# tyiannak/pyAudioAnalysis

Measured on AMD Instinct MI355X. Metric: short-term frames/sec (34-feat, 16 kHz, 50 ms/25 ms) + HBM GB/s vs peak, higher is better.
Workload: dtype f64

## Files before the change

include/paa_hip.h:

```cpp
#ifndef PAA_HIP_H
#define PAA_HIP_H

#include <stddef.h>
#include <stdint.h>

#ifdef __cplusplus
extern "C" {
#endif

#define PAA_OK                 0
#define PAA_ERR_ARG          (-1)
#define PAA_ERR_UNSUPPORTED  (-2)
#define PAA_ERR_HIP          (-3)
#define PAA_ERR_OOM          (-4)
#define PAA_ERR_TOO_SHORT    (-5)
#define PAA_ERR_CHROMA_VALUE (-6)
#define PAA_ERR_CHROMA_INDEX (-7)
#define PAA_ERR_MEL_INDEX    (-8)
#define PAA_ERR_COMM         (-9)

#define PAA_N_BASE_FEATURES 34

const char *paa_version(void);
const char *paa_last_error(void);
// ... 193 lines not shown
int paa_lda_dev_project_f64(const double *d_x, int n_dims, int64_t ld, int64_t n_vec, const double *xbar, const double *scalings,
                            int n_out, double *d_y, int64_t ld_y);

#define PAA_COMM_ID_BYTES 128
int paa_comm_unique_id(void *id_out );
int paa_comm_init(int world_size, int rank, const void *id);
int paa_comm_destroy(void);
int paa_comm_gather_f64(const double *d_send, const int64_t *counts, int root, double *d_recv);
int paa_comm_gatherv_f64(const double *d_send, const int64_t *counts, const int64_t *displs, int root, double *d_recv);
int paa_comm_barrier(void);

int paa_debug_mel_bank(double fs, int num_fft, double *out_dense);
int paa_debug_dct(double *out_13x40);
int paa_debug_chroma(double fs, int num_fft, int capacity, int32_t *src, double *weight, int32_t *slot);
int paa_debug_plan_clip_norms(paa_plan_t *plan, const void *d_packed, double *out, int64_t capacity);
int paa_debug_wave_trace(uint64_t *out, int max_waves);
int paa_debug_lane_peak(void);
int paa_debug_phase_cycles(uint64_t *out16);
int paa_debug_fft_plan(int window, int32_t *radices, int32_t *fft_len);
int paa_debug_comm_marker_name(const void *unique_id, int rank, char *out, int capacity);
int paa_debug_tri_plan(int window, double fs, int32_t *shape8, int32_t *offsets6, unsigned char *blob, int capacity);
int paa_debug_wg_plan(int window, int32_t *info32, uint16_t *perm, int perm_capacity);
int paa_debug_wgs_plan(int window, int32_t *info16, int32_t *bin_of, int capacity);
int paa_debug_wgr_tables(double fs, int window, int32_t *mel_job, int32_t *mel_fil, int32_t *ch_n, int32_t *ch_src, double *ch_w);
int paa_debug_wgr_runs(const int64_t *frames, int64_t n_clips, int num_cu, int32_t *runs3, int64_t capacity, int64_t *n_runs);
int paa_debug_blu_plan(int window, double fs, int32_t *info8, int32_t *offsets3, unsigned char *blob, int capacity);
int paa_debug_lane_jobs(const int32_t *first, const int32_t *wfirst, const int32_t *cnt, int n_owners, int32_t *jobs256);
int paa_debug_mix_plan(int window, int32_t *radices, int32_t *fft_len, uint16_t *perm, int perm_capacity,
                       int32_t *waves, int32_t *tw_global);
int paa_debug_run_plan(const int64_t *frames, int64_t n_clips, int quantum, int min_run, int max_run, int halo, int wg_runs,
// ... 11 lines not shown
```

pyaudioanalysis_amd/_ffi.py:

```python
import ctypes as C
import os
import threading

import numpy as np

from . import _build

PAA_OK = 0
ERR_ARG, ERR_UNSUPPORTED, ERR_HIP, ERR_OOM = -1, -2, -3, -4
ERR_TOO_SHORT, ERR_CHROMA_VALUE, ERR_CHROMA_INDEX, ERR_MEL_INDEX, ERR_COMM = -5, -6, -7, -8, -9
COMM_ID_BYTES = 128

_lock = threading.Lock()
_lib = None

c_i16p = C.POINTER(C.c_int16)
c_f64p = C.POINTER(C.c_double)
c_i64p = C.POINTER(C.c_int64)
c_i32p = C.POINTER(C.c_int32)


class HipLibraryError(RuntimeError):
    """libpaa_hip.so is missing / unbuildable, or the HIP runtime reported an error."""

# ... 133 lines not shown
    "paa_lda_dev_project_f64": (C.c_int, [C.c_void_p, C.c_int, C.c_int64, C.c_int64, c_f64p, c_f64p, C.c_int, C.c_void_p,
                                          C.c_int64]),
    "paa_comm_unique_id": (C.c_int, [C.c_void_p]),
    "paa_comm_init": (C.c_int, [C.c_int, C.c_int, C.c_void_p]),
    "paa_comm_destroy": (C.c_int, []),
    "paa_comm_gather_f64": (C.c_int, [C.c_void_p, c_i64p, C.c_int, C.c_void_p]),
    "paa_comm_gatherv_f64": (C.c_int, [C.c_void_p, c_i64p, c_i64p, C.c_int, C.c_void_p]),
    "paa_comm_barrier": (C.c_int, []),
    "paa_debug_mel_bank": (C.c_int, [C.c_double, C.c_int, c_f64p]),
    "paa_debug_dct": (C.c_int, [c_f64p]),
    "paa_debug_chroma": (C.c_int, [C.c_double, C.c_int, C.c_int, c_i32p, c_f64p, c_i32p]),
    "paa_debug_plan_clip_norms": (C.c_int, [C.c_void_p, C.c_void_p, c_f64p, C.c_int64]),
    "paa_debug_phase_cycles": (C.c_int, [C.POINTER(C.c_uint64)]),
    "paa_debug_wave_trace": (C.c_int, [C.POINTER(C.c_uint64), C.c_int]),
    "paa_debug_lane_peak": (C.c_int, []),
    "paa_debug_fft_plan": (C.c_int, [C.c_int, c_i32p, c_i32p]),
    "paa_debug_comm_marker_name": (C.c_int, [C.c_void_p, C.c_int, C.c_char_p, C.c_int]),
    "paa_debug_tri_plan": (C.c_int, [C.c_int, C.c_double, c_i32p, c_i32p, C.c_void_p, C.c_int]),
    "paa_debug_wg_plan": (C.c_int, [C.c_int, c_i32p, C.POINTER(C.c_uint16), C.c_int]),
    "paa_debug_wgs_plan": (C.c_int, [C.c_int, c_i32p, c_i32p, C.c_int]),
    "paa_debug_wgr_tables": (C.c_int, [C.c_double, C.c_int, c_i32p, c_i32p, c_i32p, c_i32p, c_f64p]),
    "paa_debug_wgr_runs": (C.c_int, [c_i64p, C.c_int64, C.c_int, c_i32p, C.c_int64, c_i64p]),
    "paa_debug_blu_plan": (C.c_int, [C.c_int, C.c_double, c_i32p, c_i32p, C.c_void_p, C.c_int]),
    "paa_debug_lane_jobs": (C.c_int, [c_i32p, c_i32p, c_i32p, C.c_int, c_i32p]),
    "paa_debug_mix_plan": (C.c_int, [C.c_int, c_i32p, c_i32p, C.POINTER(C.c_uint16), C.c_int, c_i32p, c_i32p]),
    "paa_debug_run_plan": (C.c_int, [c_i64p, C.c_int64, C.c_int, C.c_int, C.c_int, C.c_int, C.c_int, C.c_int, c_i32p,
                                     c_i64p, c_i32p]),
    "paa_debug_run_plan_shrink": (C.c_int, [c_i64p, C.c_int64, C.c_int, C.c_int, C.c_int, C.c_int, C.c_int, C.c_int, c_i32p,
                                     c_i64p, c_i32p]),
    "paa_debug_balanced_runs": (C.c_int64, [c_i64p, C.c_int64, C.c_int, C.c_int, C.c_int, C.c_int, C.c_int, C.c_int, c_i32p,
# ... 230 lines not shown
```

pyaudioanalysis_amd/csrc/comm_rccl.hpp:

```cpp
#pragma once
#include <dirent.h>
#include <fcntl.h>
#include <signal.h>
#include <sys/stat.h>
#include <unistd.h>

#include <rccl/rccl.h>

namespace {
struct RcclApi {
    void *h = nullptr;
    ncclResult_t (*GetUniqueId)(ncclUniqueId *) = nullptr;
    ncclResult_t (*CommInitRank)(ncclComm_t *, int, ncclUniqueId, int) = nullptr;
    ncclResult_t (*CommDestroy)(ncclComm_t) = nullptr;
    ncclResult_t (*Send)(const void *, size_t, ncclDataType_t, int, ncclComm_t, hipStream_t) = nullptr;
    ncclResult_t (*Recv)(void *, size_t, ncclDataType_t, int, ncclComm_t, hipStream_t) = nullptr;
    ncclResult_t (*GroupStart)() = nullptr;
    ncclResult_t (*GroupEnd)() = nullptr;
    ncclResult_t (*AllReduce)(const void *, void *, size_t, ncclDataType_t, ncclRedOp_t, ncclComm_t, hipStream_t) = nullptr;
    const char *(*GetErrorString)(ncclResult_t) = nullptr;
};
RcclApi g_rccl;
ncclComm_t g_comm = nullptr;
int g_world = 1, g_rank = 0;
// ... 179 lines not shown
    if (g_comm_stream) { (void)hipStreamDestroy(g_comm_stream); g_comm_stream = nullptr; }
    if (g_bar) { (void)hipFree(g_bar); g_bar = nullptr; }
    comm_release_device();
    g_world = 1;
    g_rank = 0;
    return PAA_OK;
}

extern "C" int paa_comm_gatherv_f64(const double *d_send, const int64_t *counts, const int64_t *displs, int root,
                                    double *d_recv) {
    if (!counts || !displs) return fail(PAA_ERR_ARG, "null counts / displs");
    std::lock_guard<std::mutex> lk(g_mu);
    if (!g_comm) {
        if (g_world != 1) return fail(PAA_ERR_COMM, "communicator not initialised");
        if (d_recv && d_send && d_recv + displs[0] != d_send && counts[0] > 0)
            HIP_TRY(hipMemcpyAsync(d_recv + displs[0], d_send, (size_t)counts[0] * 8, hipMemcpyDeviceToDevice, g_main_stream));
        return PAA_OK;
    }
    if (root < 0 || root >= g_world) return fail(PAA_ERR_ARG, "bad root");
    if (g_rank == root && !d_recv) return fail(PAA_ERR_ARG, "root needs a receive buffer");
    HIP_TRY(hipEventRecord(g_ev_ready, g_main_stream));
    HIP_TRY(hipStreamWaitEvent(g_comm_stream, g_ev_ready, 0));
    NCCL_TRY(g_rccl.GroupStart());
    ncclResult_t in_group = ncclSuccess;
    if (g_rank == root) {
        for (int r = 0; r < g_world && in_group == ncclSuccess; ++r)
            if (r != root && counts[r] > 0)
                in_group = g_rccl.Recv(d_recv + displs[r], (size_t)counts[r], ncclDouble, r, g_comm, g_comm_stream);
    } else if (counts[g_rank] > 0) {
        if (!d_send) in_group = ncclInvalidArgument;
        else in_group = g_rccl.Send(d_send, (size_t)counts[g_rank], ncclDouble, root, g_comm, g_comm_stream);
    }
    const ncclResult_t at_end = g_rccl.GroupEnd();
    if (in_group != ncclSuccess) return fail(PAA_ERR_COMM, "ncclSend / ncclRecv of the gather: %s", g_rccl.GetErrorString(in_group));
    if (at_end != ncclSuccess) return fail(PAA_ERR_COMM, "ncclGroupEnd of the gather: %s", g_rccl.GetErrorString(at_end));
    if (g_rank == root && d_send && counts[root] > 0 && d_recv + displs[root] != d_send)
// ... 26 lines not shown
        else (void)hipGetLastError();
        for (auto it = g_gather_done.begin(); it != g_gather_done.end();) {
            const char *k = static_cast<const char *>(it->first);
            if (k >= lo && k < hi) {
                if (it->second) gone.push_back(it->second);
                it = g_gather_done.erase(it);
            } else {
                ++it;
            }
        }
    }
    for (hipEvent_t ev : gone) { (void)hipEventSynchronize(ev); (void)hipEventDestroy(ev); }
}
static hipStream_t comm_stream_or_null() { return g_comm ? g_comm_stream : nullptr; }
static int comm_order_after_compute(hipStream_t s) {
    HIP_TRY(hipEventRecord(g_ev_ready, g_main_stream));
    HIP_TRY(hipStreamWaitEvent(s, g_ev_ready, 0));
    return PAA_OK;
}
static int comm_wait_buffer_free(const void *d_out) {
    auto it = g_gather_done.find(d_out);
    if (it != g_gather_done.end() && it->second) HIP_TRY(hipStreamWaitEvent(g_main_stream, it->second, 0));
    return PAA_OK;
}
static int comm_sync() {
    if (g_comm_stream) HIP_TRY(hipStreamSynchronize(g_comm_stream));
    return PAA_OK;
}

extern "C" int paa_comm_barrier(void) {
    if (!g_comm) return PAA_OK;
    HIP_TRY(hipStreamSynchronize(g_main_stream));
    NCCL_TRY(g_rccl.AllReduce(g_bar, g_bar, 1, ncclInt, ncclSum, g_comm, g_comm_stream));
    HIP_TRY(hipStreamSynchronize(g_comm_stream));
    return PAA_OK;
}
```

pyaudioanalysis_amd/csrc/lib_debug.hpp:

```cpp
#pragma once
extern "C" int paa_debug_phase_cycles(uint64_t *out16) {
    if (!out16) return fail(PAA_ERR_ARG, "null");
    for (int i = 0; i < 16; ++i) out16[i] = 0;
#if defined(PAA_F800_TIMING) || defined(PAA_F800_TRACE)
    int rc = ensure_init();
    if (rc) return rc;
    HIP_TRY(hipStreamSynchronize(cs()));
    unsigned long long acc[16] = {0};
    if (launch::phase_fast(acc, nullptr, 0) < 0 || launch::phase_ct(acc, nullptr, 0) < 0 || launch::phase_tri_a(acc, nullptr, 0) < 0 ||
        launch::phase_tri_b(acc, nullptr, 0) < 0 || launch::phase_tri_c(acc, nullptr, 0) < 0 || launch::phase_rmg(acc, nullptr, 0) < 0 || launch::phase_blu(acc, nullptr, 0) < 0 ||
        launch::phase_wgr(acc, nullptr, 0) < 0)
        return fail(PAA_ERR_HIP, "reading the phase counters failed");
    for (int i = 0; i < 16; ++i) out16[i] = acc[i];
#endif
    return PAA_OK;
}

extern "C" int paa_debug_lane_peak(void) {
    std::lock_guard<std::mutex> lk(g_lane_mu);
    const int p = g_lanes_peak;
    g_lanes_peak = g_lanes_active;
    return p;
}

// ... 10 lines not shown
#else
    return 0;
#endif
}

extern "C" int paa_debug_plan_clip_norms(paa_plan_t *plan, const void *d_packed, double *out, int64_t capacity) {
    if (!plan || !d_packed || !out) return fail(PAA_ERR_ARG, "null plan / buffer");
    if (capacity < 10 * (plan->n_clips + 1))
        return fail(PAA_ERR_ARG, "capacity %lld < %lld doubles", (long long)capacity, 10LL * (plan->n_clips + 1));
    { const int rc_init = ensure_init(); if (rc_init) return rc_init; }
    std::lock_guard<std::mutex> lk(g_mu);
    const int rc = launch_stats(plan, d_packed, true);
    if (rc) return rc;
    HIP_TRY(hipStreamSynchronize(cs()));
    std::vector<ClipNorm> nm((size_t)plan->n_clips);
    HIP_TRY(hipMemcpy(nm.data(), plan->d_norms, nm.size() * sizeof(ClipNorm), hipMemcpyDeviceToHost));
    const double head[10] = {(double)plan->stat_chunk, (double)g_num_cu, (double)plan->n_clips, (double)plan->n_chunks,
                             (double)plan->P.norms_inline, (double)plan->sample_kind, 0.0, 0.0, 0.0, 0.0};
    std::copy(head, head + 10, out);
    for (long long c = 0; c < plan->n_clips; ++c) {
        const ClipNorm &n = nm[(size_t)c];
        const double row[10] = {n.mean, n.inv, n.mu, n.delta_mu, (double)n.m_int, (double)n.zb, (double)n.mu_whole, n.dc_shift,
                                (double)plan->clips[c].stat_first, (double)plan->clips[c].stat_count};
        std::copy(row, row + 10, out + 10 * (c + 1));
    }
    return PAA_OK;
}

extern "C" int paa_debug_mel_bank(double fs, int num_fft, double *out_dense) {
    if (!out_dense || num_fft < 1) return fail(PAA_ERR_ARG, "bad argument");
    MelTable t;
    int rc = build_mel(fs, num_fft, t);
    if (rc) return fail(rc, "mel filter bank indexes bin >= num_fft");
    std::fill(out_dense, out_dense + (size_t)kNumMel * num_fft, 0.0);
    for (int m = 0; m < kNumMel; ++m)
        for (int i = 0; i < t.cnt[m]; ++i) out_dense[(size_t)m * num_fft + t.lo[m] + i] = t.w[t.off[m] + i];
    return PAA_OK;
}
extern "C" int paa_debug_dct(double *out_13x40) {
    if (!out_13x40) return fail(PAA_ERR_ARG, "null");
    build_dct(out_13x40);
// ... 219 lines not shown
```

pyaudioanalysis_amd/csrc/lib_dispatch.hpp:

```cpp
#pragma once

struct FamilyCtx {
    paa_plan *p;
    TableSet *tab;
    double fs;
    int window, step, deltas, mode, sample_kind, F;
    long long total_frames;
    int ranges;
    int num_cu() const { return g_num_cu * (ranges > 1 ? ranges : 1); }
    const MelTable *mel() const { return mode == 0 ? &tab->mel : nullptr; }
    const ChromaTable *chroma() const { return mode != 1 ? &tab->chroma : nullptr; }
};
struct RunRule {
    int run = 64, quantum = 4, halo_inside = 0;
    int fill_wg_runs = 0;
    int fill_min_run = 16;
};
struct Family {
    const char *id;
    int (*select)(const FamilyCtx &c, FamilyChoice &f, std::vector<unsigned char> &blob);
    int (*work)(FamilyCtx &c, std::vector<Tile> &tiles);
    int (*execute)(paa_plan *p, const void *d_packed, double *d_out, const Tile *tiles, long long n_tiles);
    bool ranged;
    bool norms_inline;
// ... 40 lines not shown
    }
}
template <void (*Rule)(FamilyCtx &, RunRule &)>
static int tile_work(FamilyCtx &c, std::vector<Tile> &tiles) {
    RunRule rr;
    Rule(c, rr);
    build_tiles(c, rr, tiles);
    return PAA_OK;
}
typedef int (*TileLaunch)(const paa_plan *p, const TileArgs &a);
template <TileLaunch Launch>
static int tile_execute(paa_plan *p, const void *d_packed, double *d_out, const Tile *tiles, long long n_tiles) {
    if (n_tiles == 0) return PAA_OK;
    ProfScope prof_scope;
    { const int rc_p = prof_scope.begin(); if (rc_p) return rc_p; }
    const TileArgs a{p->P, p->fam.d_blob, d_packed, p->sample_kind, p->d_clips, p->d_norms, tiles, n_tiles, d_out, cs()};
    return Launch(p, a) ? launch_failed(p) : PAA_OK;
}

static int fam_fast_select(const FamilyCtx &c, FamilyChoice &f, std::vector<unsigned char> &) {
    if (c.mode != 0 || g_force_generic) return 0;
    const int rc = fast_select(c.window, c.step, c.sample_kind, c.fs, c.tab->fast, c.tab->fft, c.tab->mel, c.tab->chroma, f.fl,
                               g_f800_waves);
    if (rc < 0) return fail(rc, "building the tables of the specialised kernel failed");
    if (rc) { f.lds = f.fl.lds; f.kernel_name = f.fl.name; }
    return rc;
}
static void fam_fast_rule(FamilyCtx &c, RunRule &r) {
    const FastLaunch &fl = c.p->fam.fl;
    r.quantum = 4;
    r.halo_inside = c.deltas ? 2 : 1;
// ... 158 lines not shown
                        wg::FrameRef f = p->wg_frames[(size_t)i];
                        f.halo |= q << 8;
                        p->wg_tasks.push_back(f);
                    }
            p->wg_task_chunks.emplace_back(t0, (long long)p->wg_tasks.size());
        }
    } else {
        return PAA_OK;
    }
    if (p->wg_tasks.size() > 0x7fffffffULL) return fail(PAA_ERR_UNSUPPORTED, "too many frames for the split transform");
    return upload_pooled(&p->d_wg_tasks, p->wg_tasks.data(), std::max<size_t>(p->wg_tasks.size(), 1));
}
static int fam_wgs_work(FamilyCtx &c, std::vector<Tile> &) { return wg_build_work(c.p, wgs::wgs_select(c.window).r0); }
static int fam_wg_work(FamilyCtx &c, std::vector<Tile> &) { return wg_build_work(c.p, 0); }
static WgArgs wg_args(const paa_plan *p, const void *d_packed, double *d_out) {
    return WgArgs{p->P, d_packed, p->sample_kind, p->d_clips, p->d_norms, d_out, g_num_cu, cs()};
}
static int fam_wgr_execute(paa_plan *p, const void *d_packed, double *d_out, const Tile *runs, long long n_runs) {
    return run_wgr(p, wg_args(p, d_packed, d_out), runs, n_runs);
}
static int fam_wgs_execute(paa_plan *p, const void *d_packed, double *d_out, const Tile *, long long) {
    return run_wgs(p, wg_args(p, d_packed, d_out), wgs::wgs_select(p->P.W));
}
static int fam_wg_execute(paa_plan *p, const void *d_packed, double *d_out, const Tile *, long long) {
    const WgArgs a = wg_args(p, d_packed, d_out);
    return with_sample_type(p->sample_kind, [&](auto tag) {
        typedef PAA_SAMPLE_T(tag) T;
        wg_kernel_order<T>();
        return p->fam.wl.r0 ? run_wg_split<T>(p, a) : run_wg_lds<T>(p, a);
    });
}
// ... 61 lines not shown
```

pyaudioanalysis_amd/csrc/lib_host_api.hpp:

```cpp
#pragma once
constexpr long long kRangedMinFrames = 65536;

static int run_host_st(const void *packed, const int64_t *offsets, int64_t n_clips, int sample_kind, double fs,
                       int window, int step, int deltas, double *out, const int64_t *out_offsets,
                       int64_t mid_ratio, int64_t mid_step, double *mid_out, const int64_t *mid_out_offsets) {
    if (!packed || !offsets) return fail(PAA_ERR_ARG, "null signal");
    { const int rc0 = ensure_init(); if (rc0) return rc0; }
    LaneGuard lane;
    const bool want_mid = mid_out != nullptr;
    if (want_mid && !deltas) return fail(PAA_ERR_ARG, "mid-term features are defined over the 68 delta rows");
    if (want_mid && mid_step < 1)
        return fail(PAA_ERR_ARG, "mid_step / short_step rounds to %lld: the reference loops forever "
                    "(MidTermFeatures.py:102,124)", (long long)mid_step);
    paa_plan *plan = nullptr;
    int rc;
    const long long frames_1 = (n_clips == 1) ? paa_num_frames(offsets[1] - offsets[0], window, step) : 0;
    const bool ranged = n_clips == 1 && out && !out_offsets && !want_mid && frames_1 >= kRangedMinFrames;
    {
        std::lock_guard<std::mutex> lk(g_mu);
        rc = plan_build(offsets, n_clips, sample_kind, fs, window, step, deltas, 0, &plan, ranged ? kCopyRanges : 1);
    }
    if (rc) return rc;
    std::unique_ptr<paa_plan, void (*)(paa_plan *)> guard(plan, plan_free_synced);
    const size_t esz = sample_kind == 0 ? 2 : (sample_kind == 2 ? 4 : 8);
// ... 188 lines not shown
    if (mode == 2) {
        int64_t filled = 0;
        paa_chromagram_rows(n, window, step, &filled);
        if (filled > plan->clips[0].T) {
            const long long pos = (long long)window + (long long)plan->clips[0].T * step;
            const long long last_len = n - ((long long)window + (filled - 1) * step);
            if (last_len < window / 2)
                return fail(PAA_ERR_CHROMA_VALUE, "truncated last chromagram frame shorter than num_fft "
                            "(ValueError in the reference, ShortTermFeatures.py:288)");
            const int n_tail = (int)(filled - plan->clips[0].T);
            const size_t spill = chroma_tail_spill_bytes(plan->P, n_tail);
            if (spill) {
                std::lock_guard<std::mutex> lk(g_mu);
                if ((rc = scratch_reserve(lane.l->mid, spill))) return rc;
            }
            rc = launch_chroma_tail(plan->P, sample_kind, d_samples, pos, n, n_tail, plan->d_norms,
                                    (double *)lane.l->out.p + (long long)plan->clips[0].T * 12,
                                    spill ? (double *)lane.l->mid.p : nullptr, cs());
            if (rc == -2) return fail(PAA_ERR_UNSUPPORTED, "truncated chromagram tail frame with window %d does not fit LDS", window);
            if (rc) return fail(PAA_ERR_HIP, "chromagram tail launch failed");
        }
    }
    HIP_TRY(hipMemcpyAsync(out, lane.l->out.p, (size_t)plan->out_doubles * 8, hipMemcpyDeviceToHost, cs()));
    HIP_TRY(hipStreamSynchronize(cs()));
    return PAA_OK;
}

extern "C" int paa_spectrogram_i16(const int16_t *s, int64_t n, double fs, int w, int st, double *out) {
    return run_host_spec(s, n, 0, fs, w, st, 1, out);
}
extern "C" int paa_spectrogram_f64(const double *s, int64_t n, double fs, int w, int st, double *out) {
// ... 85 lines not shown
```

pyaudioanalysis_amd/csrc/lib_plan.hpp:

```cpp
#pragma once
#ifndef PAA_STAT_CHUNK
#define PAA_STAT_CHUNK 131072
#endif
constexpr int kStatChunk = PAA_STAT_CHUNK;
static int stat_chunk_for(long long total_samples, int num_cu) {
    const long long blocks = (total_samples + kStatChunk - 1) / kStatChunk;
    if (blocks < num_cu) {
        const long long len = ((total_samples + 4LL * num_cu - 1) / (4LL * num_cu) + 63) / 64 * 64;
        return (int)std::min<long long>(kStatChunk, std::max<long long>(len, 4096));
    }
    const long long want = (blocks + num_cu - 1) / num_cu * num_cu;
    const long long len = ((total_samples + want - 1) / want + 63) / 64 * 64;
    return (int)std::min<long long>(kStatChunk, std::max<long long>(len, 4096));
}

static int choose_run_cap(const std::vector<ClipDev> &clips, int quantum, int min_run, int max_run, int halo, int wg_runs,
                          int num_cu, int shrink = 0) {
    std::map<long long, long long> hist;
    for (const ClipDev &c : clips)
        if (c.T > 0) ++hist[c.T];
    if (hist.empty()) return max_run;
    long long best_cost = -1;
    int best = max_run;
    for (int cap = max_run / quantum * quantum; cap >= min_run; cap -= quantum) {
// ... 72 lines not shown

struct FamilyChoice {
    int family = -1;
    FastLaunch fl;
    ct::CtLaunch cl;
    tri::TriLaunch trl;
    mix::MixLayout ml;
    blu::BluLayout bl;
    GenLayout gl;
    wg::WgLayout wl;
    size_t lds = 0;
    std::string kernel_name;
    unsigned char *d_blob = nullptr;
};

struct paa_plan {
    long long n_clips = 0;
    int sample_kind = 0;
    int mode = 0;
    int row_width = 0;
    std::vector<ClipDev> clips;
    std::vector<long long> alloc_rows;
    long long total_frames = 0, out_doubles = 0;
    TableSet *tab = nullptr;
    int stat_chunk = kStatChunk;
    PlanDev P;
    ClipDev *d_clips = nullptr;
    ClipNorm *d_norms = nullptr;
    Tile *d_tiles = nullptr;
    StatChunk *d_chunks = nullptr;
    void *d_psum = nullptr, *d_pmin = nullptr, *d_pmax = nullptr;
    long long *d_mid_off = nullptr;
    FamilyChoice fam;
    bool blob_cached = false;
    void *d_block = nullptr;
    void *d_big = nullptr;
    size_t big_bytes = 0;
    std::vector<wg::FrameRef> wg_frames;
    std::vector<std::pair<long long, long long>> wg_chunks;
    wg::FrameRef *d_wg_frames = nullptr;
    std::vector<wg::FrameRef> wg_tasks;
    std::vector<std::pair<long long, long long>> wg_task_chunks;
    wg::FrameRef *d_wg_tasks = nullptr;
    long long wg_rows = 0;
    long long mid_off_step = -1;
    long long n_tiles = 0, n_chunks = 0;
// ... 4 lines not shown
static void plan_free(paa_plan *p) {
    if (!p) return;
    --g_live_plans;
    pool_free(p->d_block);
    pool_free(p->d_mid_off);
    pool_free(p->d_wg_frames);
    pool_free(p->d_wg_tasks);
    if (!p->blob_cached) pool_free(p->fam.d_blob);
    if (p->d_big) (void)hipFree(p->d_big);
    delete p;
}

static void plan_free_synced(paa_plan *p) {
    if (!p) return;
    if (cs()) (void)hipStreamSynchronize(cs());
    plan_free(p);
}

static int launch_stats(paa_plan *p, const void *d_packed, bool force_params = false) {
    if (p->n_chunks > 0) {
        if (p->sample_kind == 0)
            hipLaunchKernelGGL(clip_stats_i16_kernel, dim3((unsigned)p->n_chunks), dim3(256), 0, cs(),
                               (const int16_t *)d_packed, p->d_chunks, (long long *)p->d_psum, (int *)p->d_pmin,
                               (int *)p->d_pmax);
        else if (p->sample_kind == 2)
            hipLaunchKernelGGL(clip_stats_stereo_kernel, dim3((unsigned)p->n_chunks), dim3(256), 0, cs(),
                               (const stereo16 *)d_packed, p->d_chunks, (long long *)p->d_psum, (int *)p->d_pmin,
                               (int *)p->d_pmax);
        else
            hipLaunchKernelGGL(clip_stats_f64_kernel, dim3((unsigned)p->n_chunks), dim3(256), 0, cs(),
                               (const double *)d_packed, p->d_chunks, (double *)p->d_psum, (double *)p->d_pmin,
                               (double *)p->d_pmax);
    }
    const unsigned gb = (unsigned)p->n_clips;
    if (p->P.norms_inline && !force_params) {
        HIP_TRY(hipGetLastError());
        return PAA_OK;
    }
    if (p->sample_kind == 1)
        hipLaunchKernelGGL((clip_params_kernel<double, double>), dim3(gb), dim3(64), 0, cs(), p->d_clips,
                           p->n_clips, (const double *)p->d_psum, (const double *)p->d_pmin,
                           (const double *)p->d_pmax, sample_scale<double>(), p->P.W, p->d_norms);
    else
        hipLaunchKernelGGL((clip_params_kernel<long long, int>), dim3(gb), dim3(64), 0, cs(), p->d_clips,
                           p->n_clips, (const long long *)p->d_psum, (const int *)p->d_pmin, (const int *)p->d_pmax,
                           p->sample_kind == 2 ? sample_scale<stereo16>() : sample_scale<int16_t>(), p->P.W, p->d_norms);
    HIP_TRY(hipGetLastError());
    return PAA_OK;
}

static int grow_big(paa_plan *p, size_t need, bool *fresh) {
    *fresh = false;
    if (need <= p->big_bytes) return PAA_OK;
    if (p->d_big) {
        HIP_TRY(hipStreamSynchronize(cs()));
        (void)hipFree(p->d_big);
        p->d_big = nullptr;
        p->big_bytes = 0;
    }
    HIP_TRY(hipMalloc(&p->d_big, need));
    p->big_bytes = need;
// ... 16 lines not shown
    double2 *bufA = reinterpret_cast<double2 *>(p->d_big);
    double2 *bufB = bufA + C * Nc;
    double *spec = reinterpret_cast<double *>(bufB + C * Nc);
    double *tfeat = spec + (C + 1) * Nf;
    const unsigned gx = (unsigned)std::min<long long>(64, (std::max<long long>(Nc, P.W) + 255) / 256);
    for (long long c = 0; c < p->n_clips; ++c) {
        const ClipDev &cd = p->clips[c];
        const T *x0 = (const T *)d_packed + cd.sample_off + P.frame_origin;
        double *oc = d_out + cd.out_off;
        long long prev_n = 0;
        for (long long t0 = 0; t0 < cd.T; t0 += C) {
            const long long n = std::min<long long>(C, cd.T - t0);
            if (t0 > 0 && P.mode != 1)
                HIP_TRY(hipMemcpyAsync(spec, spec + prev_n * Nf, (size_t)Nf * 8, hipMemcpyDeviceToDevice, cs()));
            hipLaunchKernelGGL(big_load_kernel<T>, dim3(gx, (unsigned)n), dim3(256), 0, cs(), P, x0, t0, ClipNorm(),
                               p->d_norms, (int)c, bufA);
            if (P.mode == 0)
                hipLaunchKernelGGL(big_time_kernel, dim3((unsigned)n), dim3(64), 0, cs(), P, bufA, tfeat);
            double2 *src = bufA, *dst = bufB;
            int Ns = 1;
            for (int q = 0; q < P.n_pass; ++q) {
                hipLaunchKernelGGL(big_pass_kernel, dim3(gx, (unsigned)n), dim3(256), 0, cs(), (int)Nc, P.radix[q], Ns,
                                   P.tw, src, dst);
                Ns *= P.radix[q];
                std::swap(src, dst);
            }
            if (P.mode == 1) {
                hipLaunchKernelGGL(big_post_kernel, dim3(gx, (unsigned)n), dim3(256), 0, cs(), P, src, oc, t0);
            } else {
                hipLaunchKernelGGL(big_post_kernel, dim3(gx, (unsigned)n), dim3(256), 0, cs(), P, src, spec, 1LL);
                hipLaunchKernelGGL(big_feat_kernel, dim3((unsigned)n), dim3(64), 0, cs(), P, spec, tfeat, t0,
// ... 22 lines not shown
            HIP_TRY(hipEventCreate(&b));
            g_prof_ev.emplace_back(a, b);
        }
        const hipEvent_t start = g_prof_ev[g_prof_used].first;
        stop = g_prof_ev[g_prof_used].second;
        ++g_prof_used;
        HIP_TRY(hipEventRecord(start, cs()));
        return PAA_OK;
    }
    void end() {
        if (stop) (void)hipEventRecord(stop, cs());
        stop = nullptr;
    }
    ~ProfScope() { end(); }
};

static int launch_failed(const paa_plan *p, const char *of = "") {
    return fail(PAA_ERR_HIP, "launch of %s%s failed: %s", of, p->fam.kernel_name.c_str(), hipGetErrorString(hipGetLastError()));
}

static int launch_wg_deltas(paa_plan *p, double *d_out) {
    if (p->P.mode != 0 || !p->P.deltas) return PAA_OK;
    long long maxT = 0;
    for (auto &cd : p->clips) maxT = std::max<long long>(maxT, cd.T);
    const long long gx = ((long long)kBase * maxT + 255) / 256;
    if (gx > 0x7fffffffLL)
        return fail(PAA_ERR_UNSUPPORTED, "delta grid too large (%lld frames in one clip)", maxT);
    for (long long c0 = 0; c0 < p->n_clips; c0 += 65535) {
        const unsigned ny = (unsigned)std::min<long long>(65535, p->n_clips - c0);
        hipLaunchKernelGGL(wg::wg_delta_kernel, dim3((unsigned)gx, ny), dim3(256), 0, cs(), p->d_clips + c0, d_out);
// ... 221 lines not shown
    std::vector<StatChunk> chunks;
    chunks.reserve((size_t)n_chunks);
    for (int64_t c = 0; c < n_clips; ++c)
        for (int i = 0; i < p->clips[c].stat_count; ++i) {
            StatChunk ch; ch.start = p->clips[c].sample_off + (long long)i * kChunk;
            ch.len = (int)std::min<long long>(kChunk, p->clips[c].n - (long long)i * kChunk);
            ch.clip = (int)c;
            chunks.push_back(ch);
        }
    {
        const size_t nch = (size_t)std::max<long long>(n_chunks, 1);
        const size_t o_clips = 0, o_tiles = o_clips + up256(p->clips.size() * sizeof(ClipDev));
        const size_t o_chunks = o_tiles + up256(std::max<size_t>(tiles.size(), 1) * sizeof(Tile));
        const size_t o_norms = o_chunks + up256(std::max<size_t>(chunks.size(), 1) * sizeof(StatChunk));
        const size_t o_sum = o_norms + up256((size_t)n_clips * sizeof(ClipNorm));
        const size_t o_min = o_sum + up256(nch * 8), o_max = o_min + up256(nch * 8), total = o_max + up256(nch * 8);
        if ((rc = pool_alloc(&p->d_block, total))) return rc;
        std::vector<unsigned char> stage(o_norms, 0);
        memcpy(stage.data() + o_clips, p->clips.data(), p->clips.size() * sizeof(ClipDev));
        if (!tiles.empty()) memcpy(stage.data() + o_tiles, tiles.data(), tiles.size() * sizeof(Tile));
        if (!chunks.empty()) memcpy(stage.data() + o_chunks, chunks.data(), chunks.size() * sizeof(StatChunk));
        HIP_TRY(hipMemcpy(p->d_block, stage.data(), o_norms, hipMemcpyHostToDevice));
        unsigned char *b = reinterpret_cast<unsigned char *>(p->d_block);
        p->d_clips = reinterpret_cast<ClipDev *>(b + o_clips);
        p->d_tiles = reinterpret_cast<Tile *>(b + o_tiles);
        p->d_chunks = reinterpret_cast<StatChunk *>(b + o_chunks);
        p->d_norms = reinterpret_cast<ClipNorm *>(b + o_norms);
        p->d_psum = b + o_sum; p->d_pmin = b + o_min; p->d_pmax = b + o_max;
    }
    P.st_sum = p->d_psum; P.st_min = p->d_pmin; P.st_max = p->d_pmax;
    P.st_scale = sample_kind == 1 ? sample_scale<double>() : (sample_kind == 2 ? sample_scale<stereo16>() : sample_scale<int16_t>());
    P.norms_inline = (fam.norms_inline && mode != 2) ? 1 : 0;
    *out = p.release();
    return PAA_OK;
}

extern "C" int paa_plan_execute(paa_plan_t *plan, const void *d_packed, double *d_out) {
    if (!plan || !d_packed || !d_out) return fail(PAA_ERR_ARG, "null plan / buffer");
    { const int rc_init = ensure_init(); if (rc_init) return rc_init; }
    std::lock_guard<std::mutex> lk(g_mu);
    int rc = comm_wait_buffer_free(d_out);
    if (rc) return rc;
    rc = launch_stats(plan, d_packed);
    if (rc) return rc;
    return kFamilies[plan->fam.family].execute(plan, d_packed, d_out, plan->d_tiles, plan->n_tiles);
}

extern "C" int paa_plan_create(const int64_t *offsets, int64_t n_clips, int sample_kind, double fs, int window,
                               int step, int deltas, paa_plan_t **out_plan) {
    std::lock_guard<std::mutex> lk(g_mu);
    return plan_build(offsets, n_clips, sample_kind, fs, window, step, deltas, 0, out_plan);
}

extern "C" int paa_plan_create_mode(const int64_t *offsets, int64_t n_clips, int sample_kind, double fs, int window,
                                    int step, int mode, paa_plan_t **out_plan) {
    if (mode < 0 || mode > 2) return fail(PAA_ERR_ARG, "mode must be 0 (features), 1 (spectrogram) or 2 (chromagram)");
    std::lock_guard<std::mutex> lk(g_mu);
    return plan_build(offsets, n_clips, sample_kind, fs, window, step, 0, mode, out_plan);
}

extern "C" int paa_plan_destroy(paa_plan_t *plan) {
    if (g_device.load() >= 0) (void)ensure_init();
    std::lock_guard<std::mutex> lk(g_mu);
    if (cs()) (void)hipStreamSynchronize(cs());
    plan_free(plan);
    return PAA_OK;
}

extern "C" int64_t paa_plan_total_frames(const paa_plan_t *plan) { return plan ? plan->total_frames : 0; }
extern "C" int64_t paa_plan_out_doubles(const paa_plan_t *plan) { return plan ? plan->out_doubles : 0; }
extern "C" const char *paa_plan_kernel_name(const paa_plan_t *plan) { return plan ? plan->fam.kernel_name.c_str() : ""; }

extern "C" int paa_plan_out_offsets(const paa_plan_t *plan, int64_t *out_offsets) {
    if (!plan || !out_offsets) return fail(PAA_ERR_ARG, "null plan / buffer");
    for (long long c = 0; c < plan->n_clips; ++c) out_offsets[c] = plan->clips[c].out_off;
    return PAA_OK;
}

extern "C" int64_t paa_plan_mid_doubles(const paa_plan_t *plan, int64_t mid_step_ratio) {
// ... 108 lines not shown
```

pyaudioanalysis_amd/csrc/paa_lib.hip:

```cpp
#include <dlfcn.h>
#include <hip/hip_runtime.h>

#include <algorithm>
#include <atomic>
#include <cstdarg>
#include <cstdio>
#include <cmath>
#include <cstring>
#include <limits>
#include <map>
#include <memory>
#include <condition_variable>
#include <mutex>
#include <string>
#include <tuple>
#include <utility>
#include <vector>

#include "../../include/paa_hip.h"
#include "family_launch.hpp"
#include "model_launch.hpp"
#include "kernels_aux.hpp"
#include "kernels_big.hpp"
#include "kernels_wg.hpp"
// ... 43 lines not shown
    size_t cap = 0;
};
struct GlobalScratch : Scratch {
    GlobalScratch *next;
    GlobalScratch();
};
static GlobalScratch *g_global_scratch = nullptr;
inline GlobalScratch::GlobalScratch() : next(g_global_scratch) { g_global_scratch = this; }

static std::mutex g_mu;
static std::mutex g_api_mu;
static std::atomic<int> g_device{-1};
static std::recursive_mutex g_init_mu;
static hipStream_t g_main_stream = nullptr;
static hipEvent_t g_ev0 = nullptr, g_ev1 = nullptr;
static std::map<std::pair<double, int>, std::unique_ptr<TableSet>> g_tables;
constexpr int kCopyRanges = 4;
struct Lane {
    hipStream_t stream = nullptr;
    hipStream_t copy_stream = nullptr;
    hipEvent_t range_done[kCopyRanges] = {nullptr, nullptr, nullptr, nullptr};
    Scratch in, out, mid;
    bool busy = false;
};
constexpr int kLanes = 4;
static Lane g_lanes[kLanes];
static std::mutex g_lane_mu;
static std::condition_variable g_lane_cv;
static int g_lanes_active = 0, g_lanes_peak = 0;
static thread_local Lane *tl_lane = nullptr;
static inline hipStream_t cs() { return tl_lane ? tl_lane->stream : g_main_stream; }
struct LaneGuard {
    Lane *l = nullptr;
    bool nested = false;
    LaneGuard() {
        if (tl_lane) { l = tl_lane; nested = true; return; }
        std::unique_lock<std::mutex> lk(g_lane_mu);
        for (;;) {
            for (int i = 0; i < kLanes; ++i)
                if (!g_lanes[i].busy && g_lanes[i].stream) { l = &g_lanes[i]; break; }
            if (l) break;
            g_lane_cv.wait(lk);
        }
        l->busy = true;
        g_lanes_peak = std::max(g_lanes_peak, ++g_lanes_active);
        tl_lane = l;
// ... 209 lines not shown
    }
    int n = 0;
    hipError_t e = hipGetDeviceCount(&n);
    if (e != hipSuccess || n < 1)
        return fail(PAA_ERR_HIP, "no HIP device (%s); this library has no CPU path", hipGetErrorString(e));
    if (device_id < 0 || device_id >= n) return fail(PAA_ERR_ARG, "device %d out of range (%d devices)", device_id, n);
    if (g_device >= 0 && g_device != device_id) {
        if (g_live_plans.load() > 0)
            return fail(PAA_ERR_ARG, "paa_init(%d): %d plan(s) of device %d are still alive; destroy them first",
                        device_id, g_live_plans.load(), g_device.load());
        paa_shutdown();
    }
    HIP_TRY(hipSetDevice(device_id));
    tl_device = device_id;
    if (!g_main_stream) HIP_TRY(hipStreamCreateWithFlags(&g_main_stream, hipStreamNonBlocking));
    for (int i = 0; i < kLanes; ++i) {
        if (!g_lanes[i].stream) HIP_TRY(hipStreamCreateWithFlags(&g_lanes[i].stream, hipStreamNonBlocking));
        if (!g_lanes[i].copy_stream) HIP_TRY(hipStreamCreateWithFlags(&g_lanes[i].copy_stream, hipStreamNonBlocking));
        for (int k = 0; k < kCopyRanges; ++k)
            if (!g_lanes[i].range_done[k]) HIP_TRY(hipEventCreateWithFlags(&g_lanes[i].range_done[k], hipEventDisableTiming));
    }
    if (!g_ev0) HIP_TRY(hipEventCreate(&g_ev0));
    if (!g_ev1) HIP_TRY(hipEventCreate(&g_ev1));
    {
        int ncu = 0;
        if (hipDeviceGetAttribute(&ncu, hipDeviceAttributeMultiprocessorCount, device_id) == hipSuccess && ncu > 0) g_num_cu = ncu;
    }
    const char *fg = experiment_env("PAA_HIP_FORCE_GENERIC");
    g_force_generic = (fg && fg[0] == '1') ? 1 : 0;
    const char *fw = experiment_env("PAA_F800_WAVES");
    g_f800_waves = (fw && fw[0] == '4') ? 4 : 8;
    g_device.store(device_id, std::memory_order_release);
    return PAA_OK;
}

extern "C" void paa_shutdown(void) {
    std::lock_guard<std::recursive_mutex> init_lock(g_init_mu);
    if (g_device < 0) return;
    (void)paa_comm_destroy();
    if (g_main_stream) (void)hipStreamSynchronize(g_main_stream);
    for (auto &kv : g_tables) free_tables(*kv.second);
    g_tables.clear();
    pool_release_all();
    for (GlobalScratch *s = g_global_scratch; s; s = s->next) scratch_release(*s);
    for (Lane &ln : g_lanes) {
        if (ln.stream) { (void)hipStreamSynchronize(ln.stream); (void)hipStreamDestroy(ln.stream); ln.stream = nullptr; }
        if (ln.copy_stream) { (void)hipStreamSynchronize(ln.copy_stream); (void)hipStreamDestroy(ln.copy_stream); ln.copy_stream = nullptr; }
        for (hipEvent_t &ev : ln.range_done) { if (ev) (void)hipEventDestroy(ev); ev = nullptr; }
        for (Scratch *s : {&ln.in, &ln.out, &ln.mid}) scratch_release(*s);
    }
    if (g_ev0) (void)hipEventDestroy(g_ev0);
    if (g_ev1) (void)hipEventDestroy(g_ev1);
    if (g_main_stream) (void)hipStreamDestroy(g_main_stream);
    g_ev0 = g_ev1 = nullptr;
    g_main_stream = nullptr;
    ++lds_attr_generation();
    g_device.store(-1, std::memory_order_release);
}

extern "C" int paa_dev_alloc(size_t bytes, void **out_ptr) {
    int rc = ensure_init();
    if (rc) return rc;
    if (!out_ptr) return fail(PAA_ERR_ARG, "null out_ptr");
    HIP_TRY(hipMalloc(out_ptr, bytes ? bytes : 1));
    return PAA_OK;
}
extern "C" int paa_dev_free(void *ptr) {
    if (ptr) {
        comm_forget_buffer(ptr);
        HIP_TRY(hipFree(ptr));
// ... 20 lines not shown
    HIP_TRY(hipMemcpyAsync(dst, src, bytes, hipMemcpyDeviceToHost, cs()));
    HIP_TRY(hipStreamSynchronize(cs()));
    return PAA_OK;
}
extern "C" int paa_memcpy_d2h_compute(void *dst, const void *src, size_t bytes) {
    int rc = ensure_init();
    if (rc) return rc;
    HIP_TRY(hipMemcpyAsync(dst, src, bytes, hipMemcpyDeviceToHost, cs()));
    HIP_TRY(hipStreamSynchronize(cs()));
    return PAA_OK;
}
extern "C" int paa_dev_sync(void) {
    int rc = ensure_init();
    if (rc) return rc;
    HIP_TRY(hipStreamSynchronize(cs()));
    return comm_sync();
}
extern "C" int paa_timer_start(void) {
    int rc = ensure_init();
    if (rc) return rc;
    HIP_TRY(hipEventRecord(g_ev0, cs()));
    return PAA_OK;
}
extern "C" int paa_timer_stop(float *ms) {
    int rc = ensure_init();
    if (rc) return rc;
    HIP_TRY(hipEventRecord(g_ev1, cs()));
    HIP_TRY(hipEventSynchronize(g_ev1));
    HIP_TRY(hipEventElapsedTime(ms, g_ev0, g_ev1));
    return PAA_OK;
// ... 71 lines not shown
```

Baseline: 573.1 million.

## Overlap per-clip stats kernels on a side stream with previous feature execution

```diff
diff --git a/include/paa_hip.h b/include/paa_hip.h
--- a/include/paa_hip.h
+++ b/include/paa_hip.h
@@ -231,6 +231,7 @@
 int paa_debug_dct(double *out_13x40);
 int paa_debug_chroma(double fs, int num_fft, int capacity, int32_t *src, double *weight, int32_t *slot);
 int paa_debug_plan_clip_norms(paa_plan_t *plan, const void *d_packed, double *out, int64_t capacity);
+int paa_debug_stats_overlap(int mode, int64_t *counters2);
 int paa_debug_wave_trace(uint64_t *out, int max_waves);
 int paa_debug_lane_peak(void);
 int paa_debug_phase_cycles(uint64_t *out16);
diff --git a/pyaudioanalysis_amd/_ffi.py b/pyaudioanalysis_amd/_ffi.py
--- a/pyaudioanalysis_amd/_ffi.py
+++ b/pyaudioanalysis_amd/_ffi.py
@@ -171,6 +171,7 @@
     "paa_debug_phase_cycles": (C.c_int, [C.POINTER(C.c_uint64)]),
     "paa_debug_wave_trace": (C.c_int, [C.POINTER(C.c_uint64), C.c_int]),
     "paa_debug_lane_peak": (C.c_int, []),
+    "paa_debug_stats_overlap": (C.c_int, [C.c_int, c_i64p]),
     "paa_debug_fft_plan": (C.c_int, [C.c_int, c_i32p, c_i32p]),
     "paa_debug_comm_marker_name": (C.c_int, [C.c_void_p, C.c_int, C.c_char_p, C.c_int]),
     "paa_debug_tri_plan": (C.c_int, [C.c_int, C.c_double, c_i32p, c_i32p, C.c_void_p, C.c_int]),
diff --git a/pyaudioanalysis_amd/csrc/comm_rccl.hpp b/pyaudioanalysis_amd/csrc/comm_rccl.hpp
--- a/pyaudioanalysis_amd/csrc/comm_rccl.hpp
+++ b/pyaudioanalysis_amd/csrc/comm_rccl.hpp
@@ -217,12 +217,12 @@
     if (!g_comm) {
         if (g_world != 1) return fail(PAA_ERR_COMM, "communicator not initialised");
         if (d_recv && d_send && d_recv + displs[0] != d_send && counts[0] > 0)
-            HIP_TRY(hipMemcpyAsync(d_recv + displs[0], d_send, (size_t)counts[0] * 8, hipMemcpyDeviceToDevice, g_main_stream));
+            HIP_TRY(hipMemcpyAsync(d_recv + displs[0], d_send, (size_t)counts[0] * 8, hipMemcpyDeviceToDevice, main_q()));
         return PAA_OK;
     }
     if (root < 0 || root >= g_world) return fail(PAA_ERR_ARG, "bad root");
     if (g_rank == root && !d_recv) return fail(PAA_ERR_ARG, "root needs a receive buffer");
-    HIP_TRY(hipEventRecord(g_ev_ready, g_main_stream));
+    HIP_TRY(hipEventRecord(g_ev_ready, main_q()));
     HIP_TRY(hipStreamWaitEvent(g_comm_stream, g_ev_ready, 0));
     NCCL_TRY(g_rccl.GroupStart());
     ncclResult_t in_group = ncclSuccess;
@@ -279,13 +279,13 @@
 }
 static hipStream_t comm_stream_or_null() { return g_comm ? g_comm_stream : nullptr; }
 static int comm_order_after_compute(hipStream_t s) {
-    HIP_TRY(hipEventRecord(g_ev_ready, g_main_stream));
+    HIP_TRY(hipEventRecord(g_ev_ready, main_q()));
     HIP_TRY(hipStreamWaitEvent(s, g_ev_ready, 0));
     return PAA_OK;
 }
 static int comm_wait_buffer_free(const void *d_out) {
     auto it = g_gather_done.find(d_out);
-    if (it != g_gather_done.end() && it->second) HIP_TRY(hipStreamWaitEvent(g_main_stream, it->second, 0));
+    if (it != g_gather_done.end() && it->second) HIP_TRY(hipStreamWaitEvent(main_q(), it->second, 0));
     return PAA_OK;
 }
 static int comm_sync() {
diff --git a/pyaudioanalysis_amd/csrc/lib_debug.hpp b/pyaudioanalysis_amd/csrc/lib_debug.hpp
--- a/pyaudioanalysis_amd/csrc/lib_debug.hpp
+++ b/pyaudioanalysis_amd/csrc/lib_debug.hpp
@@ -48,7 +48,7 @@
     if (rc) return rc;
     HIP_TRY(hipStreamSynchronize(cs()));
     std::vector<ClipNorm> nm((size_t)plan->n_clips);
-    HIP_TRY(hipMemcpy(nm.data(), plan->d_norms, nm.size() * sizeof(ClipNorm), hipMemcpyDeviceToHost));
+    HIP_TRY(hipMemcpy(nm.data(), plan->st[0].norms, nm.size() * sizeof(ClipNorm), hipMemcpyDeviceToHost));
     const double head[10] = {(double)plan->stat_chunk, (double)g_num_cu, (double)plan->n_clips, (double)plan->n_chunks,
                              (double)plan->P.norms_inline, (double)plan->sample_kind, 0.0, 0.0, 0.0, 0.0};
     std::copy(head, head + 10, out);
@@ -59,6 +59,14 @@
         std::copy(row, row + 10, out + 10 * (c + 1));
     }
     return PAA_OK;
+}
+
+extern "C" int paa_debug_stats_overlap(int mode, int64_t *counters2) {
+    std::lock_guard<std::mutex> lk(g_mu);
+    const int was = g_stat_overlap;
+    if (mode >= 0 && mode <= 2) g_stat_overlap = mode;
+    if (counters2) { counters2[0] = g_ov_taken; counters2[1] = g_ov_fallback; }
+    return was;
 }
 
 extern "C" int paa_debug_mel_bank(double fs, int num_fft, double *out_dense) {
diff --git a/pyaudioanalysis_amd/csrc/lib_dispatch.hpp b/pyaudioanalysis_amd/csrc/lib_dispatch.hpp
--- a/pyaudioanalysis_amd/csrc/lib_dispatch.hpp
+++ b/pyaudioanalysis_amd/csrc/lib_dispatch.hpp
@@ -78,7 +78,9 @@
     if (n_tiles == 0) return PAA_OK;
     ProfScope prof_scope;
     { const int rc_p = prof_scope.begin(); if (rc_p) return rc_p; }
-    const TileArgs a{p->P, p->fam.d_blob, d_packed, p->sample_kind, p->d_clips, p->d_norms, tiles, n_tiles, d_out, cs()};
+    PlanDev P = p->P;
+    const ClipNorm *norms = plan_launch_set(p, P);
+    const TileArgs a{P, p->fam.d_blob, d_packed, p->sample_kind, p->d_clips, norms, tiles, n_tiles, d_out, cs()};
     return Launch(p, a) ? launch_failed(p) : PAA_OK;
 }
 
@@ -267,7 +269,7 @@
 static int fam_wgs_work(FamilyCtx &c, std::vector<Tile> &) { return wg_build_work(c.p, wgs::wgs_select(c.window).r0); }
 static int fam_wg_work(FamilyCtx &c, std::vector<Tile> &) { return wg_build_work(c.p, 0); }
 static WgArgs wg_args(const paa_plan *p, const void *d_packed, double *d_out) {
-    return WgArgs{p->P, d_packed, p->sample_kind, p->d_clips, p->d_norms, d_out, g_num_cu, cs()};
+    return WgArgs{p->P, d_packed, p->sample_kind, p->d_clips, p->st[0].norms, d_out, g_num_cu, cs()};
 }
 static int fam_wgr_execute(paa_plan *p, const void *d_packed, double *d_out, const Tile *runs, long long n_runs) {
     return run_wgr(p, wg_args(p, d_packed, d_out), runs, n_runs);
diff --git a/pyaudioanalysis_amd/csrc/lib_host_api.hpp b/pyaudioanalysis_amd/csrc/lib_host_api.hpp
--- a/pyaudioanalysis_amd/csrc/lib_host_api.hpp
+++ b/pyaudioanalysis_amd/csrc/lib_host_api.hpp
@@ -226,7 +226,7 @@
                 std::lock_guard<std::mutex> lk(g_mu);
                 if ((rc = scratch_reserve(lane.l->mid, spill))) return rc;
             }
-            rc = launch_chroma_tail(plan->P, sample_kind, d_samples, pos, n, n_tail, plan->d_norms,
+            rc = launch_chroma_tail(plan->P, sample_kind, d_samples, pos, n, n_tail, plan->st[0].norms,
                                     (double *)lane.l->out.p + (long long)plan->clips[0].T * 12,
                                     spill ? (double *)lane.l->mid.p : nullptr, cs());
             if (rc == -2) return fail(PAA_ERR_UNSUPPORTED, "truncated chromagram tail frame with window %d does not fit LDS", window);
diff --git a/pyaudioanalysis_amd/csrc/lib_plan.hpp b/pyaudioanalysis_amd/csrc/lib_plan.hpp
--- a/pyaudioanalysis_amd/csrc/lib_plan.hpp
+++ b/pyaudioanalysis_amd/csrc/lib_plan.hpp
@@ -110,6 +110,11 @@
     unsigned char *d_blob = nullptr;
 };
 
+struct StatSet {
+    void *psum = nullptr, *pmin = nullptr, *pmax = nullptr;
+    ClipNorm *norms = nullptr;
+};
+
 struct paa_plan {
     long long n_clips = 0;
     int sample_kind = 0;
@@ -122,10 +127,12 @@
     int stat_chunk = kStatChunk;
     PlanDev P;
     ClipDev *d_clips = nullptr;
-    ClipNorm *d_norms = nullptr;
     Tile *d_tiles = nullptr;
     StatChunk *d_chunks = nullptr;
-    void *d_psum = nullptr, *d_pmin = nullptr, *d_pmax = nullptr;
+    StatSet st[2];
+    int run_set = -1;
+    bool used_side = false;
+    long long in_lo = 0, in_hi = 0;
     long long *d_mid_off = nullptr;
     FamilyChoice fam;
     bool blob_cached = false;
@@ -160,23 +167,26 @@
 static void plan_free_synced(paa_plan *p) {
     if (!p) return;
     if (cs()) (void)hipStreamSynchronize(cs());
+    if (p->used_side) (void)stat_stream_sync();
     plan_free(p);
 }
 
-static int launch_stats(paa_plan *p, const void *d_packed, bool force_params = false) {
+static int launch_stats(paa_plan *p, const void *d_packed, bool force_params = false, bool side = false, int set = 0) {
+    const hipStream_t s = side ? g_stat_stream : cs();
+    const StatSet &st = p->st[set];
     if (p->n_chunks > 0) {
         if (p->sample_kind == 0)
-            hipLaunchKernelGGL(clip_stats_i16_kernel, dim3((unsigned)p->n_chunks), dim3(256), 0, cs(),
-                               (const int16_t *)d_packed, p->d_chunks, (long long *)p->d_psum, (int *)p->d_pmin,
-                               (int *)p->d_pmax);
+            hipLaunchKernelGGL(clip_stats_i16_kernel, dim3((unsigned)p->n_chunks), dim3(256), 0, s,
+                               (const int16_t *)d_packed, p->d_chunks, (long long *)st.psum, (int *)st.pmin,
+                               (int *)st.pmax);
         else if (p->sample_kind == 2)
-            hipLaunchKernelGGL(clip_stats_stereo_kernel, dim3((unsigned)p->n_chunks), dim3(256), 0, cs(),
-                               (const stereo16 *)d_packed, p->d_chunks, (long long *)p->d_psum, (int *)p->d_pmin,
-                               (int *)p->d_pmax);
+            hipLaunchKernelGGL(clip_stats_stereo_kernel, dim3((unsigned)p->n_chunks), dim3(256), 0, s,
+                               (const stereo16 *)d_packed, p->d_chunks, (long long *)st.psum, (int *)st.pmin,
+                               (int *)st.pmax);
         else
-            hipLaunchKernelGGL(clip_stats_f64_kernel, dim3((unsigned)p->n_chunks), dim3(256), 0, cs(),
-                               (const double *)d_packed, p->d_chunks, (double *)p->d_psum, (double *)p->d_pmin,
-                               (double *)p->d_pmax);
+            hipLaunchKernelGGL(clip_stats_f64_kernel, dim3((unsigned)p->n_chunks), dim3(256), 0, s,
+                               (const double *)d_packed, p->d_chunks, (double *)st.psum, (double *)st.pmin,
+                               (double *)st.pmax);
     }
     const unsigned gb = (unsigned)p->n_clips;
     if (p->P.norms_inline && !force_params) {
@@ -184,13 +194,13 @@
         return PAA_OK;
     }
     if (p->sample_kind == 1)
-        hipLaunchKernelGGL((clip_params_kernel<double, double>), dim3(gb), dim3(64), 0, cs(), p->d_clips,
-                           p->n_clips, (const double *)p->d_psum, (const double *)p->d_pmin,
-                           (const double *)p->d_pmax, sample_scale<double>(), p->P.W, p->d_norms);
+        hipLaunchKernelGGL((clip_params_kernel<double, double>), dim3(gb), dim3(64), 0, s, p->d_clips,
+                           p->n_clips, (const double *)st.psum, (const double *)st.pmin,
+                           (const double *)st.pmax, sample_scale<double>(), p->P.W, st.norms);
     else
-        hipLaunchKernelGGL((clip_params_kernel<long long, int>), dim3(gb), dim3(64), 0, cs(), p->d_clips,
-                           p->n_clips, (const long long *)p->d_psum, (const int *)p->d_pmin, (const int *)p->d_pmax,
-                           p->sample_kind == 2 ? sample_scale<stereo16>() : sample_scale<int16_t>(), p->P.W, p->d_norms);
+        hipLaunchKernelGGL((clip_params_kernel<long long, int>), dim3(gb), dim3(64), 0, s, p->d_clips,
+                           p->n_clips, (const long long *)st.psum, (const int *)st.pmin, (const int *)st.pmax,
+                           p->sample_kind == 2 ? sample_scale<stereo16>() : sample_scale<int16_t>(), p->P.W, st.norms);
     HIP_TRY(hipGetLastError());
     return PAA_OK;
 }
@@ -237,7 +247,7 @@
             if (t0 > 0 && P.mode != 1)
                 HIP_TRY(hipMemcpyAsync(spec, spec + prev_n * Nf, (size_t)Nf * 8, hipMemcpyDeviceToDevice, cs()));
             hipLaunchKernelGGL(big_load_kernel<T>, dim3(gx, (unsigned)n), dim3(256), 0, cs(), P, x0, t0, ClipNorm(),
-                               p->d_norms, (int)c, bufA);
+                               p->st[0].norms, (int)c, bufA);
             if (P.mode == 0)
                 hipLaunchKernelGGL(big_time_kernel, dim3((unsigned)n), dim3(64), 0, cs(), P, bufA, tfeat);
             double2 *src = bufA, *dst = bufB;
@@ -290,6 +300,14 @@
     }
     ~ProfScope() { end(); }
 };
+
+static const ClipNorm *plan_launch_set(const paa_plan *p, PlanDev &P) {
+    if (p->run_set < 0) return p->st[0].norms;
+    const StatSet &st = p->st[p->run_set];
+    P.st_sum = st.psum; P.st_min = st.pmin; P.st_max = st.pmax;
+    P.norms_inline = (g_stat_overlap == 2) ? 1 : 0;
+    return st.norms;
+}
 
 static int launch_failed(const paa_plan *p, const char *of = "") {
     return fail(PAA_ERR_HIP, "launch of %s%s failed: %s", of, p->fam.kernel_name.c_str(), hipGetErrorString(hipGetLastError()));
@@ -541,7 +559,8 @@
         const size_t o_chunks = o_tiles + up256(std::max<size_t>(tiles.size(), 1) * sizeof(Tile));
         const size_t o_norms = o_chunks + up256(std::max<size_t>(chunks.size(), 1) * sizeof(StatChunk));
         const size_t o_sum = o_norms + up256((size_t)n_clips * sizeof(ClipNorm));
-        const size_t o_min = o_sum + up256(nch * 8), o_max = o_min + up256(nch * 8), total = o_max + up256(nch * 8);
+        const size_t o_min = o_sum + up256(nch * 8), o_max = o_min + up256(nch * 8), o_set1 = o_max + up256(nch * 8);
+        const size_t set_bytes = o_set1 - o_norms, total = o_set1 + set_bytes;
         if ((rc = pool_alloc(&p->d_block, total))) return rc;
         std::vector<unsigned char> stage(o_norms, 0);
         memcpy(stage.data() + o_clips, p->clips.data(), p->clips.size() * sizeof(ClipDev));
@@ -552,13 +571,50 @@
         p->d_clips = reinterpret_cast<ClipDev *>(b + o_clips);
         p->d_tiles = reinterpret_cast<Tile *>(b + o_tiles);
         p->d_chunks = reinterpret_cast<StatChunk *>(b + o_chunks);
-        p->d_norms = reinterpret_cast<ClipNorm *>(b + o_norms);
-        p->d_psum = b + o_sum; p->d_pmin = b + o_min; p->d_pmax = b + o_max;
-    }
-    P.st_sum = p->d_psum; P.st_min = p->d_pmin; P.st_max = p->d_pmax;
+        for (int k = 0; k < 2; ++k) {
+            unsigned char *bs = b + k * set_bytes;
+            p->st[k].norms = reinterpret_cast<ClipNorm *>(bs + o_norms);
+            p->st[k].psum = bs + o_sum; p->st[k].pmin = bs + o_min; p->st[k].pmax = bs + o_max;
+        }
+    }
+    {
+        const long long esz = sample_kind == 0 ? 2 : (sample_kind == 2 ? 4 : 8);
+        p->in_lo = (long long)offsets[0] * esz;
+        p->in_hi = (long long)offsets[n_clips] * esz;
+    }
+    P.st_sum = p->st[0].psum; P.st_min = p->st[0].pmin; P.st_max = p->st[0].pmax;
     P.st_scale = sample_kind == 1 ? sample_scale<double>() : (sample_kind == 2 ? sample_scale<stereo16>() : sample_scale<int16_t>());
     P.norms_inline = (fam.norms_inline && mode != 2) ? 1 : 0;
     *out = p.release();
+    return PAA_OK;
+}
+
+static int execute_overlapped(paa_plan *plan, const void *d_packed, double *d_out) {
+    OverlapState &o = g_overlap;
+    const int slot = (int)(o.k % kStatRing), set = (int)(o.k & 1);
+    const char *in_lo = (const char *)d_packed + plan->in_lo, *in_hi = (const char *)d_packed + plan->in_hi;
+    const bool ahead = o.noted && o.epoch == g_main_epoch.load(std::memory_order_relaxed) && o.before &&
+                       !(in_lo < o.out_hi && o.out_lo < in_hi);
+    o.noted = false;
+    ++o.k;
+    ++(ahead ? g_ov_taken : g_ov_fallback);
+    const hipEvent_t e_k = g_ev_main[slot], s_k = g_ev_stat[slot];
+    HIP_TRY(hipEventRecord(e_k, g_main_stream));
+    HIP_TRY(hipStreamWaitEvent(g_stat_stream, ahead ? o.before : e_k, 0));
+    plan->used_side = true;
+    int rc = launch_stats(plan, d_packed, g_stat_overlap != 2, true, set);
+    if (rc) return rc;
+    HIP_TRY(hipEventRecord(s_k, g_stat_stream));
+    HIP_TRY(hipStreamWaitEvent(g_main_stream, s_k, 0));
+    plan->run_set = set;
+    rc = kFamilies[plan->fam.family].execute(plan, d_packed, d_out, plan->d_tiles, plan->n_tiles);
+    plan->run_set = -1;
+    if (rc) return rc;
+    o.before = e_k;
+    o.out_lo = (const char *)d_out;
+    o.out_hi = o.out_lo + plan->out_doubles * 8;
+    o.epoch = g_main_epoch.load(std::memory_order_relaxed);
+    o.noted = true;
     return PAA_OK;
 }
 
@@ -568,6 +624,8 @@
     std::lock_guard<std::mutex> lk(g_mu);
     int rc = comm_wait_buffer_free(d_out);
     if (rc) return rc;
+    if (g_stat_overlap && !tl_lane && plan->P.norms_inline && g_stat_stream) return execute_overlapped(plan, d_packed, d_out);
+    ++g_ov_fallback;
     rc = launch_stats(plan, d_packed);
     if (rc) return rc;
     return kFamilies[plan->fam.family].execute(plan, d_packed, d_out, plan->d_tiles, plan->n_tiles);
@@ -590,6 +648,7 @@
     if (g_device.load() >= 0) (void)ensure_init();
     std::lock_guard<std::mutex> lk(g_mu);
     if (cs()) (void)hipStreamSynchronize(cs());
+    (void)stat_stream_sync();
     plan_free(plan);
     return PAA_OK;
 }
diff --git a/pyaudioanalysis_amd/csrc/paa_lib.hip b/pyaudioanalysis_amd/csrc/paa_lib.hip
--- a/pyaudioanalysis_amd/csrc/paa_lib.hip
+++ b/pyaudioanalysis_amd/csrc/paa_lib.hip
@@ -81,6 +81,20 @@
 static std::recursive_mutex g_init_mu;
 static hipStream_t g_main_stream = nullptr;
 static hipEvent_t g_ev0 = nullptr, g_ev1 = nullptr;
+constexpr int kStatRing = 4;
+static hipStream_t g_stat_stream = nullptr;
+static hipEvent_t g_ev_main[kStatRing] = {nullptr, nullptr, nullptr, nullptr}, g_ev_stat[kStatRing] = {nullptr, nullptr, nullptr, nullptr};
+static std::atomic<unsigned long long> g_main_epoch{0};
+static int g_stat_overlap = 1;
+static long long g_ov_taken = 0, g_ov_fallback = 0;
+struct OverlapState {
+    unsigned long long k = 0;
+    bool noted = false;
+    unsigned long long epoch = 0;
+    hipEvent_t before = nullptr;
+    const char *out_lo = nullptr, *out_hi = nullptr;
+};
+static OverlapState g_overlap;
 static std::map<std::pair<double, int>, std::unique_ptr<TableSet>> g_tables;
 constexpr int kCopyRanges = 4;
 struct Lane {
@@ -96,7 +110,15 @@
 static std::condition_variable g_lane_cv;
 static int g_lanes_active = 0, g_lanes_peak = 0;
 static thread_local Lane *tl_lane = nullptr;
-static inline hipStream_t cs() { return tl_lane ? tl_lane->stream : g_main_stream; }
+static inline hipStream_t main_q() {
+    g_main_epoch.fetch_add(1, std::memory_order_relaxed);
+    return g_main_stream;
+}
+static inline hipStream_t cs() { return tl_lane ? tl_lane->stream : main_q(); }
+static int stat_stream_sync() {
+    if (g_stat_stream) HIP_TRY(hipStreamSynchronize(g_stat_stream));
+    return PAA_OK;
+}
 struct LaneGuard {
     Lane *l = nullptr;
     bool nested = false;
@@ -336,6 +358,15 @@
     HIP_TRY(hipSetDevice(device_id));
     tl_device = device_id;
     if (!g_main_stream) HIP_TRY(hipStreamCreateWithFlags(&g_main_stream, hipStreamNonBlocking));
+    if (!g_stat_stream) HIP_TRY(hipStreamCreateWithFlags(&g_stat_stream, hipStreamNonBlocking));
+    {
+        unsigned ring_flags = hipEventDisableTiming | hipEventDisableSystemFence;
+        if (experiment_env("PAA_STATS_EVENT_FENCE")) ring_flags = hipEventDisableTiming;
+        for (int i = 0; i < kStatRing; ++i) {
+            if (!g_ev_main[i]) HIP_TRY(hipEventCreateWithFlags(&g_ev_main[i], ring_flags));
+            if (!g_ev_stat[i]) HIP_TRY(hipEventCreateWithFlags(&g_ev_stat[i], ring_flags));
+        }
+    }
     for (int i = 0; i < kLanes; ++i) {
         if (!g_lanes[i].stream) HIP_TRY(hipStreamCreateWithFlags(&g_lanes[i].stream, hipStreamNonBlocking));
         if (!g_lanes[i].copy_stream) HIP_TRY(hipStreamCreateWithFlags(&g_lanes[i].copy_stream, hipStreamNonBlocking));
@@ -352,6 +383,7 @@
     g_force_generic = (fg && fg[0] == '1') ? 1 : 0;
     const char *fw = experiment_env("PAA_F800_WAVES");
     g_f800_waves = (fw && fw[0] == '4') ? 4 : 8;
+    if (const char *so = experiment_env("PAA_STATS_OVERLAP")) g_stat_overlap = (so[0] == '0') ? 0 : (so[0] == '2' ? 2 : 1);
     g_device.store(device_id, std::memory_order_release);
     return PAA_OK;
 }
@@ -361,6 +393,7 @@
     if (g_device < 0) return;
     (void)paa_comm_destroy();
     if (g_main_stream) (void)hipStreamSynchronize(g_main_stream);
+    if (g_stat_stream) (void)hipStreamSynchronize(g_stat_stream);
     for (auto &kv : g_tables) free_tables(*kv.second);
     g_tables.clear();
     pool_release_all();
@@ -373,9 +406,16 @@
     }
     if (g_ev0) (void)hipEventDestroy(g_ev0);
     if (g_ev1) (void)hipEventDestroy(g_ev1);
+    for (int i = 0; i < kStatRing; ++i) {
+        if (g_ev_main[i]) (void)hipEventDestroy(g_ev_main[i]);
+        if (g_ev_stat[i]) (void)hipEventDestroy(g_ev_stat[i]);
+        g_ev_main[i] = g_ev_stat[i] = nullptr;
+    }
+    if (g_stat_stream) (void)hipStreamDestroy(g_stat_stream);
     if (g_main_stream) (void)hipStreamDestroy(g_main_stream);
     g_ev0 = g_ev1 = nullptr;
-    g_main_stream = nullptr;
+    g_main_stream = g_stat_stream = nullptr;
+    g_overlap = OverlapState();
     ++lds_attr_generation();
     g_device.store(-1, std::memory_order_release);
 }
@@ -426,6 +466,7 @@
     int rc = ensure_init();
     if (rc) return rc;
     HIP_TRY(hipStreamSynchronize(cs()));
+    if (!tl_lane) { const int rc_s = stat_stream_sync(); if (rc_s) return rc_s; }
     return comm_sync();
 }
 extern "C" int paa_timer_start(void) {
```

Result: slower. 565.9 million (-1.3%).
